# AdamCodd/local-hyperDB

Measured on AMD Instinct MI355X. Metric: queries/sec, N=10M d=384 fp16 top-100 (single-query stream; p50 latency alongside), higher is better.
Workload: dtype f16; 1 GPU; N=10000000 d=384 fp16 Q=1 cosine_similarity top-100, row-sharded x1; rows_per_gpu=10000000, accumulate=f32, exchange=none

## Files before the change

### local-hyperdb_amd/csrc/hdb_api.hip

```cpp
#include "hdb_common.h"
#include "hdb_quant.h"
#include "hdb_ws.h"
#include "hdb_plan.h"
#include "hdb_group_plan.h"
#include "hdb_devbuf.h"
#include "../../include/hyperdb_hip.h"
#include <string>
#include <cmath>
#include <cstring>
#include <cstdio>
#include <algorithm>
#include <vector>
#include <chrono>
#include <atomic>

static thread_local std::string g_err;
static int fail(int code, const std::string& msg) { g_err = msg; return code; }
#define HIP_TRY(expr)                                                                              \
    do {                                                                                           \
        hipError_t e_ = (expr);                                                                    \
        if (e_ != hipSuccess)                                                                      \
            return fail(HDB_ERR_HIP, std::string(#expr) + ": " + hipGetErrorString(e_));           \
    } while (0)
#define LAUNCH_TRY(expr)                                                                           \
// ... 101 lines not shown
struct CacheBufs { DevBuf<float> inv, sq; };
static int caches_alloc(int64_t rows, CacheBufs& c) {
    HIP_TRY(c.inv.alloc((size_t)rows));
    HIP_TRY(c.sq.alloc((size_t)rows));
    return HDB_OK;
}
static void caches_commit(hdb_index* ix, CacheBufs& c) {
    if (!c.inv) return;
    ix->inv_norm.swap(c.inv); ix->sqnorm.swap(c.sq);
}

static double quant_gamma(int d) {
    const double u = std::ldexp(1.0, -24), m = (double)(d + 8) * u;
    return m / (1.0 - m) * (1.0 + std::ldexp(1.0, -20));
}
static double quant_gamma_m(int d) { return (double)(d + 8) * std::ldexp(1.0, -22); }
static double quant_gamma_rows(int d) { return std::max(quant_gamma(d), quant_gamma_m(d)); }
static size_t row_pitch(const hdb_index* ix) { return (size_t)hdb_row_bytes(ix->dtype, ix->d); }
#define HDB_QSTAT_WORDS 4
static hipError_t qstat_alloc(hdb_index* ix, hipStream_t st) {
    if (ix->qstat) return hipSuccess;
    const hipError_t e = ix->qstat.alloc(HDB_QSTAT_WORDS);
    return e != hipSuccess ? e : hipMemsetAsync(ix->qstat, 0, HDB_QSTAT_WORDS * sizeof(int), st);
}
static void plane_free(hdb_index* ix) { ix->pnib.reset(); ix->pbit.reset(); ix->prec.reset(); }
static void quant_free(hdb_index* ix) {
    ix->qcodes.reset(); ix->qaux.reset(); ix->q_rows = 0;
    plane_free(ix);
}
static size_t plane_row_bytes(int P) { return (size_t)hdb_quant_plane_units(P) * 20 + 16; }
static bool plane_alloc(hdb_index* ix, int64_t rows) {
    const size_t U = (size_t)hdb_quant_plane_units(ix->qP);
    DevBuf<uint8_t> nib; DevBuf<uint32_t> bit; DevBuf<float> rec;
    if (nib.alloc((size_t)rows * U * 16) != hipSuccess || bit.alloc((size_t)rows * U) != hipSuccess || rec.alloc((size_t)rows * 4) != hipSuccess) {
        (void)hipGetLastError();
        return false;
    }
    ix->pnib.swap(nib); ix->pbit.swap(bit); ix->prec.swap(rec);
    return true;
}
static int plane_rows(hdb_index* ix, int64_t row0, int64_t m, hipStream_t st) {
    if (!plane_possible(ix->d) || ix->plane_declined) return HDB_OK;
    if (!ix->pnib && !plane_wanted(ix->d, ix->opt)) return HDB_OK;
    if (!ix->pnib) {
        size_t free_b = 0, total_b = 0;
        if (hipMemGetInfo(&free_b, &total_b) != hipSuccess) { (void)hipGetLastError(); ix->plane_declined = true; return HDB_OK; }
        if (free_b < (size_t)ix->q_rows * plane_row_bytes(ix->qP) + ((size_t)1 << 30)) { ix->plane_declined = true; return HDB_OK; }
        if (!plane_alloc(ix, ix->q_rows)) { ix->plane_declined = true; return HDB_OK; }
        ix->pU = hdb_quant_plane_units(ix->qP);
        m = row0 + m; row0 = 0;
    }
    LAUNCH_TRY(hdb_launch_quant_plane_rows(ix->qcodes, ix->qaux, row0, m, ix->d, ix->qP, ix->pnib, ix->pbit, ix->prec, st));
    return HDB_OK;
}
struct ShadowBufs { DevBuf<int8_t> codes; DevBuf<float> aux; int64_t rows = 0; };
static int quant_alloc(const hdb_index* ix, int64_t rows, ShadowBufs& s) {
    hipError_t e = s.codes.alloc((size_t)rows * ix->qP);
    if (e == hipSuccess) e = s.aux.alloc((size_t)rows * 3);
    if (e != hipSuccess) return fail(HDB_ERR_NOMEM, std::string("the int8 shadow: ") + hipGetErrorString(e));
    s.rows = rows;
    return HDB_OK;
}
static int quant_room(const hdb_index* ix, int64_t need, bool tight, ShadowBufs& s) {
    if (need <= ix->q_rows && ix->qcodes) return HDB_OK;
    return quant_alloc(ix, tight ? need + 64 : need + need / 2 + 64, s);
}
static void quant_commit(hdb_index* ix, ShadowBufs& s) {
    if (!s.rows) return;
    ix->qcodes.swap(s.codes); ix->qaux.swap(s.aux); ix->q_rows = s.rows;
    plane_free(ix);
}
static int quant_reserve(hdb_index* ix, int64_t need, int64_t keep, hipStream_t st, bool tight = false) {
    ShadowBufs s;
    const int rc = quant_room(ix, need, tight, s);
    if (rc || !s.rows) return rc;
    if (keep > 0 && ix->qcodes) {
        HIP_TRY(hipMemcpyAsync(s.codes, ix->qcodes, (size_t)keep * ix->qP, hipMemcpyDeviceToDevice, st));
        HIP_TRY(hipMemcpyAsync(s.aux, ix->qaux, (size_t)keep * 3 * sizeof(float), hipMemcpyDeviceToDevice, st));
    }
    quant_commit(ix, s);
    return HDB_OK;
}
static int quant_rows(hdb_index* ix, int64_t row0, int64_t m, hipStream_t st) {
    if (m <= 0) return HDB_OK;
    const char* src = (const char*)ix->V + (size_t)row0 * row_pitch(ix);
// ... 1511 lines not shown
```

### local-hyperdb_amd/csrc/hdb_caps.h

```cpp
#pragma once
#include "../../include/hyperdb_hip.h"

static inline int hdb_scan_auto_blocks(int dtype, int row_bytes, bool vec, bool wide_rows) {
    if ((dtype == HDB_F8E4M3 || dtype == HDB_I8) && vec && (row_bytes == 256 || row_bytes == 384 || row_bytes == 512)) {
        const int b = 512 * 768 / row_bytes;
        return b < 1024 ? b : 1024;
    }
    return wide_rows ? 256 : 512;
}

#define HDB_BSCAN_TABLE_BYTES (60 * 1024)
static inline int hdb_bscan_qt(int d) {
    if (d <= 0 || d % 32 != 0) return -1;
    for (int qt = 4; qt >= 1; qt >>= 1)
        if ((int64_t)qt * 16 * d <= HDB_BSCAN_TABLE_BYTES) return qt;
    return (int64_t)8 * d <= HDB_BSCAN_TABLE_BYTES ? 0 : -1;
}
static inline int hdb_bscan_lds_bytes(int d, int qt) { return qt > 0 ? qt * 16 * d : 8 * d; }
static inline int hdb_bscan_auto_blocks(int d, int qt, int cus) {
    int per_cu = (160 * 1024) / (hdb_bscan_lds_bytes(d, qt) + 5 * 1024);
    per_cu = per_cu < 1 ? 1 : per_cu > 8 ? 8 : per_cu;
    return per_cu * (cus > 0 ? cus : 1);
}

// ... 206 lines not shown
    if (max_blocks > 0 && max_blocks < limit) limit = max_blocks;
    return hdb_grid_for((nwalk + 1) / 2, 4, (int)limit);
}
static inline int hdb_quant_plane_dbg_blocks(int64_t ntiles, int max_blocks) { return hdb_grid_for((ntiles + 1) / 2, 4, max_blocks > 0 ? max_blocks : 1024); }
struct HdbSkipPos { uint32_t w, o; };
struct HdbSkipStep { uint32_t dw, dn, step; };
__host__ __device__ __forceinline__ uint32_t hdb_plane_skip_count(uint32_t ntiles, uint32_t s_tiles) { return ntiles - s_tiles; }
__host__ __device__ __forceinline__ HdbSkipStep hdb_plane_skip_step(uint32_t step, uint32_t stride) {
    const uint32_t m = stride - 1u;
    HdbSkipStep s;
    s.dw = m ? step / m : 0u; s.dn = m ? step % m : 0u; s.step = step;
    return s;
}
__host__ __device__ __forceinline__ HdbSkipPos hdb_plane_skip_start(uint32_t tp, uint32_t s_tiles, uint32_t stride) {
    const uint32_t m = stride - 1u;
    HdbSkipPos p;
    const uint32_t w = m ? tp / m : s_tiles;
    if (w < s_tiles) { p.w = w; p.o = tp - w * m; }
    else { p.w = s_tiles; p.o = tp - s_tiles * m; }
    return p;
}
__host__ __device__ __forceinline__ void hdb_plane_skip_advance(HdbSkipPos& p, const HdbSkipStep& s, uint32_t s_tiles, uint32_t stride) {
    if (p.w >= s_tiles) { p.o += s.step; return; }
    const uint32_t m = stride - 1u;
    p.w += s.dw; p.o += s.dn;
    if (p.o >= m) { p.o -= m; ++p.w; }
    if (p.w >= s_tiles) { p.o += (p.w - s_tiles) * m; p.w = s_tiles; }
}
__host__ __device__ __forceinline__ int64_t hdb_plane_skip_tile(const HdbSkipPos& p, uint32_t s_tiles, uint32_t stride) {
    if (p.w >= s_tiles) return (int64_t)s_tiles * stride + p.o;
    const uint32_t jit = (uint32_t)(hdb_tile_index((int64_t)p.w, (int64_t)stride) - (int64_t)p.w * stride);
    return (int64_t)p.w * stride + p.o + (p.o >= jit ? 1u : 0u);
}

static inline int hdb_qb_supported(int d) { return d == 128 || d == 256 || d == 384 || d == 512; }
static inline void qb_shape(int nq, int& wq, int& nqt) {
    const int tq = (nq + 15) / 16;
    wq = tq <= 4 ? 1 : tq <= 8 ? 2 : 4;
    nqt = (tq + wq - 1) / wq;
}
static inline int hdb_qb_scan_blocks(int64_t ntiles, int nq, int cus, int max_blocks) {
    int wq, nqt; qb_shape(nq, wq, nqt);
    const int64_t lim = max_blocks > 0 ? max_blocks : 2 * (int64_t)cus;
    return hdb_grid_for(ntiles, 4 / wq, (int)(lim < 512 ? lim : 512));
}
static inline int64_t hdb_qb_slots(int blocks, int nq) { int wq, nqt; qb_shape(nq, wq, nqt); return (int64_t)blocks * (4 / wq) * 4; }
```

### local-hyperdb_amd/csrc/hdb_launch.h

```cpp
#pragma once
#include <stddef.h>
#include <stdint.h>

struct ScanArgs;
struct FusedArgs;
struct BatchArgs;
struct BitsArgs;
struct QuantArgs;

#define HDB_ANYD_DECL(name) int name(const ScanArgs* args, int dpad, int mode, int nq_launch, const void* q, const float* sqnorm, \
                                     const float* qsq, const float* qscl, int blocks, void* stream)
#define HDB_GEOM_DECL(name) int name(const ScanArgs* args, int mode, int nq_launch, const void* q16, const float* sqnorm, \
                                     const float* qsq, const float* qscl, int blocks, int variant, void* stream, const BatchArgs* f)

extern "C" {
int hdb_launch_scan(const ScanArgs* args, int dtype, int mode, int nq_launch, int max_blocks, void* stream);
int hdb_launch_list_rows(unsigned long long* cand, const uint32_t* cnt, uint32_t cap, int nq, const int64_t* rows, int64_t m, void* stream);
int hdb_launch_rownorm(const void* V, int64_t n, int d, int dtype, float* inv_norm, float* sqnorm, int* nan_flag, void* stream);
int hdb_launch_qprep(const void* Q, int nq, int d, bool f64, float* qinv, float* qsq, int* qnan, void* q16, float* qscl, void* stream);
int hdb_launch_qprep2(const void* Q, int nq, int d, bool f64, float* qinv, float* qsq, int* qnan, void* q16, float* qscl,
                      float* thr_init, uint32_t* cnt_init, uint32_t* qbits, int W, void* stream);
int hdb_launch_signpack(const void* V, int64_t n, int d, int dtype, int64_t row0, uint32_t* bits, void* stream);
int hdb_launch_qsign(const void* Q, int nq, int d, bool f64, int W, uint32_t* qbits, void* stream);
int hdb_launch_hamming(const ScanArgs* args, int mode, int nq_launch, const uint32_t* bits, int64_t npad, int W,
// ... 74 lines not shown
int hdb_launch_mfma_kslice_bf16(const ScanArgs* a, int dslice, int mode, int nq_launch, const void* q, const float* sqnorm,
                                const float* qsq, int blocks, void* stream);
int hdb_launch_mfma_kslice_bf16_wide(const ScanArgs* a, int dslice, int mode, int nq_launch, const void* q, const float* sqnorm,
                                     const float* qsq, int blocks, void* stream);
int hdb_launch_mfma_kslice_f8(const ScanArgs* a, int dslice, int mode, int nq_launch, const void* q, const float* sqnorm,
                              const float* qsq, int blocks, void* stream);
int hdb_launch_mfma_kslice_f8_wide(const ScanArgs* a, int dslice, int mode, int nq_launch, const void* q, const float* sqnorm,
                                   const float* qsq, int blocks, void* stream);
int hdb_launch_mfma_scan_f8_lds(const ScanArgs* args, int mode, int nq_launch, const void* q, const float* sqnorm,
                                const float* qsq, int blocks, void* stream);
int hdb_launch_mfma_scan_f8_lds_wide(const ScanArgs* args, int mode, int nq_launch, const void* q, const float* sqnorm,
                                     const float* qsq, int blocks, void* stream);
int hdb_launch_mfma_kslice_f8_lds(const ScanArgs* a, int dslice, int mode, int nq_launch, const void* q, const float* sqnorm,
                                  const float* qsq, int blocks, void* stream);
int hdb_launch_mfma_kslice_f8_lds_wide(const ScanArgs* a, int dslice, int mode, int nq_launch, const void* q, const float* sqnorm,
                                       const float* qsq, int blocks, void* stream);
HDB_ANYD_DECL(hdb_launch_mfma_anyd_a); HDB_ANYD_DECL(hdb_launch_mfma_anyd_b);
HDB_ANYD_DECL(hdb_launch_mfma_anyd_c); HDB_ANYD_DECL(hdb_launch_mfma_anyd_d);
HDB_ANYD_DECL(hdb_launch_mfma_anyd_e); HDB_ANYD_DECL(hdb_launch_mfma_anyd_f);

size_t hdb_mfma_fused_ctl_bytes(void);
int hdb_launch_mfma_fused(const ScanArgs* args, int dtype, const FusedArgs* fa, int max_blocks, void* stream);
int hdb_launch_mfma_fused_wide(const ScanArgs* args, const FusedArgs* fa, int blocks, void* stream);
int hdb_launch_bits_fused(const BitsArgs* args, int jaccard, int max_blocks, void* stream);
int hdb_launch_l1_tile(const ScanArgs* args, int dtype, int mode, int nq_launch, int max_blocks, void* stream);

int hdb_launch_quant_rows(const void* V, int64_t n, int d, int dtype, int P, int8_t* codes, float* aux, int* nan_flag, double gamma,
                          void* stream);
int hdb_launch_quant_gather(const int8_t* codes, const float* aux, const int64_t* rows, int64_t m, int P, int8_t* codes_out,
                            float* aux_out, void* stream);
int hdb_launch_quant_qprep(const float* Q, int nq, int d, int P, int8_t* qcodes, float* qaux, int* stat, uint32_t* pl_cnt, void* stream);
int hdb_launch_quant_qprep_m(const float* Q, int nq, int d, int P, float* qinv, float* qsq, int* qnan, void* q16, float* qscl,
                             int8_t* qcodes, float* qaux, int* stat, uint32_t* cnt_init, uint32_t* pl_cnt, void* stream);
int hdb_launch_quant_plane_rows(const int8_t* codes, const float* aux, int64_t row0, int64_t m, int d, int P, uint8_t* nib, uint32_t* bitw,
                                float* rec, void* stream);
int hdb_launch_quant_plane_scan(const QuantArgs* args, int dbg, int blocks, void* stream);
int hdb_launch_quant_scan(const QuantArgs* args, int mode, int max_blocks, void* stream);
int hdb_launch_quant_scan_one(const QuantArgs* args, int mode, int max_blocks, void* stream);
int hdb_launch_quant_rescore(const void* V, int d, int dtype, const float* Q, int nq, int metric, const float* inv_norm,
                             const float* qinv, const float* bias, const uint8_t* mask, unsigned long long* cand,
                             const uint32_t* cnt, uint32_t cap, void* stream);
int hdb_launch_quant_finalize(const unsigned long long* cand, const uint32_t* cnt, uint32_t cap, int nq, uint32_t k, uint32_t kk,
                              int64_t row_base, int64_t* idx_out, float* score_out, int32_t* status, const int* qnan,
                              const float* qaux, const float* thr, int* stat, unsigned long long* cand_rw, const float* sc, int64_t ld,
                              void* stream);

int hdb_launch_rerank_prep(const int64_t* cand, int m, int nq, int64_t n, int64_t row_base, const uint8_t* mask, const int* qnan,
                           int64_t* rows, uint32_t* cnt, int32_t* status, void* stream);
int hdb_launch_rerank_score(const ScanArgs* args, int dtype, int nq_launch, void* stream);

int hdb_launch_group_collapse(const int64_t* idx, const float* score, int nq, int m, int k, const int32_t* groups, int64_t n_groups,
                              int64_t n, int64_t row_base, int64_t* idx_out, float* score_out, const int32_t* status_in,
                              int32_t* status_out, int carry, void* stream);
int hdb_launch_group_best(const float* scores, int64_t n, int64_t ld, int nq, const int32_t* groups, int64_t n_groups,
                          unsigned long long* best, void* stream);
int hdb_launch_group_demote(float* scores, int64_t n, int64_t ld, int nq, const int32_t* groups, int64_t n_groups,
                            const unsigned long long* best, int* bad, void* stream);
int hdb_launch_group_finish(int64_t* idx, const float* score, int nq, int k, int32_t* status, const int* bad, void* stream);

int hdb_launch_qb_scan(const QuantArgs* args, int mode, float* wstat, int64_t wld, int max_blocks, void* stream);
int hdb_launch_qb_thr(const float* vals, int64_t n, int64_t ld, int nq, uint32_t m, float* thr, void* stream);
int hdb_launch_qb_rescore(const void* V, int d, const void* q16, const float* qscl, const float* qinv, const float* inv_norm,
                          const float* bias, const uint8_t* mask, int metric, unsigned long long* cand, const uint32_t* cnt,
                          uint32_t cap, int nq, void* stream);
}
```

### local-hyperdb_amd/csrc/hdb_quant.hip

```cpp
#include "hdb_common.h"
#include "hdb_quant.h"
#include "hdb_finalize.h"
#include "../../include/hyperdb_hip.h"

__device__ __forceinline__ float hq_up(double x) {
    x = x * (1.0 + 0x1p-40);
    float f = (float)x;
    if ((double)f < x) f = nextafterf(f, INFINITY);
    return f;
}

__device__ __forceinline__ float hq_f(__half v) { return __half2float(v); }
__device__ __forceinline__ float hq_f(hdb_bf16 v) { return hdb_bf16_to_f(v); }
__device__ __forceinline__ float hq_f(float v) { return v; }

template <typename T> struct HqElem;
template <> struct HqElem<__half> { static constexpr int EPC = 8; };
template <> struct HqElem<hdb_bf16> { static constexpr int EPC = 8; };
template <> struct HqElem<float> { static constexpr int EPC = 4; };

__device__ __forceinline__ void hq_unpack(const uint4& raw, float (&x)[8], __half*) {
    const __half2* h = reinterpret_cast<const __half2*>(&raw);
#pragma unroll
    for (int i = 0; i < 4; ++i) { float2 f = __half22float2(h[i]); x[2 * i] = f.x; x[2 * i + 1] = f.y; }
// ... 461 lines not shown
        const int64_t r0 = hdb_tile_index(t, a.tile_stride) * 16 + 4 * g;
        const int64_t rr[4] = {r0, r0 + 1, r0 + 2, r0 + 3};
        const int u_own = hdb_owned_row(l16);
        const int64_t row = r0 + u_own;
        const int64_t out_i = t * 16 + 4 * g + u_own;
        const bool live = hq_rows4_bounds<NQ, NJ, (NJ > 0 ? NJ : 2)>(a, qs, qc, rr, l16, row, [&](int q, float lo, float hi, bool masked) {
            if (MODE == 2) {
                a.dbg[row] = hi;
            } else if (MODE == 0) {
                if (a.nsub > 0) wbest[q] = max(wbest[q], hdb_f2key(lo));
                else a.scores[(int64_t)q * a.ld + out_i] = lo;
                if (NQ == 1 && a.pl_hi) a.pl_hi[out_i] = hi;
            } else if (!masked && !qc.bad[q] && hi >= q_thr[q]) {
                hq_emit(stage, q, hi, row);
            }
        });
        if (MODE == 0 && a.nsub == 0 && !live && (l16 & 3) == 0)
#pragma unroll
            for (int q = 0; q < NQ; ++q) a.scores[(int64_t)q * a.ld + out_i] = -INFINITY;
        if (MODE == 0 && NQ == 1 && a.pl_hi && !live && (l16 & 3) == 0) a.pl_hi[out_i] = -INFINITY;
    }
    if (MODE == 0 && a.nsub > 0) {
#pragma unroll
        for (int q = 0; q < NQ; ++q) {
            uint32_t wm = wbest[q];
#pragma unroll
            for (int o = 32; o > 0; o >>= 1) wm = max(wm, (uint32_t)__shfl_xor((int)wm, o, 64));
            if (lane == 0) a.wmax[(int64_t)q * a.nsub + blockIdx.x * 4 + wave] = wm;
        }
    }
    if (MODE == 1) hq_stage_flush<NQ>(stage);
}

__global__ __launch_bounds__(256) void hdb_quant_plane_rows_kernel(const int8_t* codes, const float* aux, int64_t row0, int64_t m, int d, int P,
                                                                   int U, uint8_t* nib, uint32_t* bitw, float* rec) {
    const int lane = threadIdx.x & 63, g = lane >> 4, l16 = lane & 15;
    const int64_t wave = ((int64_t)blockIdx.x * 256 + threadIdx.x) >> 6;
    const int64_t nwaves = ((int64_t)gridDim.x * 256) >> 6;
    for (int64_t base = wave * 4; base < m; base += nwaves * 4) {
        const int64_t r = row0 + base + g;
        const bool valid = base + g < m;
        int ss = 0;
        if (valid && l16 < U) {
            const int8_t* src = codes + r * (int64_t)P + 32 * l16;
            uint4 raw[2];
            raw[0] = *reinterpret_cast<const uint4*>(src);
            raw[1] = (32 * l16 + 16 < P) ? *reinterpret_cast<const uint4*>(src + 16) : make_uint4(0u, 0u, 0u, 0u);
            const uint32_t* cw = reinterpret_cast<const uint32_t*>(raw);
            uint32_t nw[4] = {0u, 0u, 0u, 0u}, bw = 0u;
#pragma unroll
            for (int w = 0; w < 8; ++w) {
#pragma unroll
                for (int b = 0; b < 4; ++b) {
                    const int c = (int)(int8_t)((cw[w] >> (8 * b)) & 0xFFu);
                    const int h = c >> 3;
                    const uint32_t u5 = (uint32_t)(h + 16);
                    const int rho = c - (8 * h + 4);
                    if (32 * l16 + 4 * w + b < d) ss += rho * rho;
                    nw[w >> 1] |= (u5 >> 1) << (8 * b + 4 * (w & 1));
                    bw |= (u5 & 1u) << (8 * b + w);
                }
            }
            *reinterpret_cast<uint4*>(nib + (r * (int64_t)U + l16) * 16) = make_uint4(nw[0], nw[1], nw[2], nw[3]);
            bitw[r * (int64_t)U + l16] = bw;
        }
#pragma unroll
        for (int o = 8; o > 0; o >>= 1) ss += __shfl_xor(ss, o, 64);
        if (valid && l16 == 0) {
            const float R = sqrtf((float)ss) * (1.f + 0x1p-20f);
            *reinterpret_cast<float4*>(rec + 4 * r) = make_float4(aux[3 * r + HDB_QROW_S], aux[3 * r + HDB_QROW_E], aux[3 * r + HDB_QROW_T], R);
        }
    }
}

#define HQ_PL_QUEUE 48
template <int J, bool DBG>
__global__ __launch_bounds__(256) __attribute__((amdgpu_num_sgpr(96))) void hdb_quant_plane_scan_kernel(QuantArgs a) {
    extern __shared__ __attribute__((aligned(16))) char smem[];
    int4* qs = reinterpret_cast<int4*>(smem);
    __shared__ int part[4][2][64 * J];
    __shared__ HqStage stage;
    __shared__ uint32_t queue[4][HQ_PL_QUEUE];
    __shared__ uint32_t surv_cnt;
    const int U = a.pl_units, nch = a.P >> 4;
    if (threadIdx.x < 4) stage.cnt[threadIdx.x] = 0u;
    if (threadIdx.x == 0) surv_cnt = 0u;
    for (int i = threadIdx.x; i < 2 * U; i += 256) qs[i] = i < nch ? reinterpret_cast<const int4*>(a.qcodes)[i] : make_int4(0, 0, 0, 0);
    const float* qo = a.qaux;
    const float q_s = qo[HDB_QQ_S], q_n = qo[HDB_QQ_N], q_d = qo[HDB_QQ_D], q_cn = qo[HDB_QQ_CN];
    const int q_cs = (int)qo[HDB_QQ_CS];
    const bool q_bad = qo[HDB_QQ_BAD] != 0.f;
    const bool cosine = a.metric == HDB_COSINE;
    const float q_inv = cosine ? a.qinv[0] : 1.f;
    float thr1[1] = {(!DBG && a.nsub == 0) ? a.thr[0] : 0.f};
    __syncthreads();
    if (!DBG && a.nsub > 0) hq_fold_thr<1>(a, thr1);
    const float q_thr = thr1[0];

    const int lane = threadIdx.x & 63, wave = __builtin_amdgcn_readfirstlane(threadIdx.x >> 6);
    const int npieces = 16 * U;
    int qoff[J];
#pragma unroll
    for (int j = 0; j < J; ++j) {
        const int f = lane + 64 * j;
        qoff[j] = f < npieces ? 2 * (f % U) : 0;
    }
    const float absmin = 0x1p-100f * (float)(a.d + 8);
    typedef unsigned int u32x4 __attribute__((ext_vector_type(4)));
    typedef float f32x4 __attribute__((ext_vector_type(4)));
    const int64_t ntiles = a.ntiles;
    const int et = lane >> 4, er = lane & 15;
    int qn = 0;
    uint32_t nsurv = 0u;
    auto drain = [&](int base, int m) {
        const QuantArgs& a = hq_args_in_memory();
        HqQuery<1> qc;
        qc.s[0] = q_s; qc.n[0] = q_n; qc.d[0] = q_d; qc.sq[0] = 0.f; qc.inv[0] = q_inv; qc.bad[0] = q_bad;
        int ln = lane;
        asm volatile("" : "+v"(ln));
        const int g = ln >> 4, l16 = ln & 15;
        int64_t rr[4];
#pragma unroll
        for (int u = 0; u < 4; ++u) rr[u] = 4 * g + u < m ? (int64_t)queue[wave][base + 4 * g + u] : a.n;
        const int own = 4 * g + hdb_owned_row(l16);
        const int64_t row = own < m ? (int64_t)queue[wave][base + own] : a.n;
        hq_rows4_bounds<1, 0, 1>(a, qs, qc, rr, l16, row, [&](int, float, float hi, bool masked) {
            if (!masked && !q_bad && hi >= q_thr) hq_emit(stage, 0, hi, row);
        });
    };

    const uint32_t s_tiles = DBG ? 0u : a.pl_s_tiles, s_stride = DBG ? 1u : a.pl_s_stride;
    const uint32_t nwalk = hdb_plane_skip_count((uint32_t)ntiles, s_tiles);
    const uint32_t tp0 = ((uint32_t)blockIdx.x * 4u + (uint32_t)wave) * 2u;
    const HdbSkipStep sk_step = hdb_plane_skip_step((uint32_t)gridDim.x * 8u, s_stride), sk_next = {0u, 1u, 1u};
    HdbSkipPos pos = hdb_plane_skip_start(tp0 < nwalk ? tp0 : 0u, s_tiles, s_stride);
    for (uint32_t tp = tp0; tp < nwalk; tp += (uint32_t)gridDim.x * 8u, hdb_plane_skip_advance(pos, sk_step, s_tiles, s_stride)) {
        int64_t tl[2];
        {
            HdbSkipPos p1 = pos;
            hdb_plane_skip_advance(p1, sk_next, s_tiles, s_stride);
            tl[0] = hdb_plane_skip_tile(pos, s_tiles, s_stride);
            tl[1] = tp + 1u < nwalk ? hdb_plane_skip_tile(p1, s_tiles, s_stride) : ntiles;
        }
        u32x4 nv[2][J];
        uint32_t bv[2][J];
        int ln = lane;
        asm volatile("" : "+v"(ln));
#pragma unroll
        for (int tt = 0; tt < 2; ++tt) {
            const int pieces_left = (int)min((int64_t)16, max((int64_t)0, a.n - tl[tt] * 16)) * U;
            const uint8_t* nb = a.pl_nib + tl[tt] * (int64_t)npieces * 16;
            const uint32_t* bb = a.pl_bit + tl[tt] * (int64_t)npieces;
#pragma unroll
            for (int j = 0; j < J; ++j) {
                if (ln < pieces_left - 64 * j) {
                    nv[tt][j] = __builtin_nontemporal_load(reinterpret_cast<const u32x4*>(nb + (uint32_t)ln * 16u) + 64 * j);
                    bv[tt][j] = __builtin_nontemporal_load(bb + (uint32_t)ln + 64 * j);
                } else {
                    nv[tt][j] = u32x4{0u, 0u, 0u, 0u};
                    bv[tt][j] = 0u;
                }
            }
        }
        const int64_t row = (et ? tl[1] : tl[0]) * 16 + er;
        const bool rvalid = lane < 32 && row < a.n;
        f32x4 rc = f32x4{0.f, 0.f, 0.f, 0.f};
        float invn = 1.f, bias = 0.f;
        bool masked = false;
        if (rvalid) {
            rc = __builtin_nontemporal_load(reinterpret_cast<const f32x4*>(a.pl_rec) + row);
            if (cosine) invn = a.inv_norm[row];
            if (a.bias) bias = a.bias[row];
            if (a.mask) masked = !a.mask[row];
        }
        __builtin_amdgcn_sched_barrier(0);
#pragma unroll
        for (int j = 0; j < J; ++j) {
            const int4 x = qs[qoff[j]], y = qs[qoff[j] + 1];
            const int qw[8] = {x.x, x.y, x.z, x.w, y.x, y.y, y.z, y.w};
#pragma unroll
            for (int tt = 0; tt < 2; ++tt) {
                const uint32_t bw = bv[tt][j];
                const uint32_t w4[4] = {nv[tt][j].x, nv[tt][j].y, nv[tt][j].z, nv[tt][j].w};
                int s = 0;
#pragma unroll
                for (int i = 0; i < 4; ++i) {
                    const uint32_t lo = ((w4[i] << 1) & 0x1E1E1E1Eu) | ((bw >> (2 * i)) & 0x01010101u);
                    const uint32_t hi = ((w4[i] >> 3) & 0x1E1E1E1Eu) | ((bw >> (2 * i + 1)) & 0x01010101u);
                    s = __builtin_amdgcn_sdot4((int)lo, qw[2 * i], s, false);
                    s = __builtin_amdgcn_sdot4((int)hi, qw[2 * i + 1], s, false);
                }
                part[wave][tt][lane + 64 * j] = s;
            }
            __builtin_amdgcn_sched_barrier(0);
        }
        __builtin_amdgcn_fence(__ATOMIC_RELEASE, "wavefront");
        __builtin_amdgcn_wave_barrier();
        __builtin_amdgcn_fence(__ATOMIC_ACQUIRE, "wavefront");
        int S = 0;
        if (lane < 32)
            for (int i = 0; i < U; ++i) S += part[wave][et][er * U + i];
        __builtin_amdgcn_fence(__ATOMIC_RELEASE, "wavefront");
        __builtin_amdgcn_wave_barrier();
        float hi5 = -INFINITY;
        const bool dead = !rvalid || masked || q_bad;
        if (!dead) {
            const float fc = (float)(8 * S - 124 * q_cs);
            const float Uf = q_cn * rc.w;
            float ch = fc + Uf, cl = fc - Uf;
            ch = ch + (fabsf(ch) * 0x1p-20f + 1.f);
            cl = cl - (fabsf(cl) * 0x1p-20f + 1.f);
            const float k = q_s * rc.x;
            const float A5 = k * ch, Al = k * cl;
            const float Amax = fmaxf(fabsf(A5), fabsf(Al));
            const float c0 = (q_n * rc.y + q_d * rc.z) * (1.f + 0x1p-10f);
            const float B5 = c0 + fabsf(A5) * 0x1p-10f + absmin;
            const float Bmax = c0 + Amax * 0x1p-10f + absmin;
            const float Mx = Amax + Bmax;
            float X = (A5 + B5) + (Mx * 0x1p-18f + 1e-30f);
            float mM = Mx * (1.f + 0x1p-17f);
            if (cosine) { X = X * invn * q_inv; mM = mM * invn * q_inv; }
            const float Z = mM + fabsf(bias);
            float h = X;
            if (a.bias) h += bias;
            hi5 = h + (Z * 0x1p-18f + 4e-30f);
            if (hi5 != hi5) hi5 = INFINITY;
        }
        if (DBG) {
            if (rvalid) a.dbg[row] = hi5;
            continue;
        }
        const bool keep = !dead && !(hi5 < q_thr);
        const unsigned long long km = __ballot(keep);
        if (km == 0ull) continue;
        if (keep) queue[wave][qn + __popcll(km & ((1ull << lane) - 1ull))] = (uint32_t)row;
        const int nk = __popcll(km);
        qn += nk; nsurv += (uint32_t)nk;
        __builtin_amdgcn_fence(__ATOMIC_RELEASE, "wavefront");
        __builtin_amdgcn_wave_barrier();
        __builtin_amdgcn_fence(__ATOMIC_ACQUIRE, "wavefront");
        if (qn >= 16) {
            do { qn -= 16; drain(qn, 16); } while (qn >= 16);
            __builtin_amdgcn_fence(__ATOMIC_RELEASE, "wavefront");
            __builtin_amdgcn_wave_barrier();
        }
    }
    if (!DBG) {
        if (s_tiles != 0u) {
            const QuantArgs& am = hq_args_in_memory();
            const uint32_t nslots = s_tiles * 16u, dslot = (uint32_t)gridDim.x * 256u;
            uint32_t cbase = ((uint32_t)blockIdx.x * 4u + (uint32_t)wave) * 64u;
            float hnext = cbase + lane < nslots ? am.pl_hi[cbase + lane] : 0.f;
#pragma unroll 1
            for (; cbase < nslots; cbase += dslot) {
// ... 166 lines not shown
    const int nch = a.P >> 4;
    const int nj = (nch + 15) >> 4;
    if (nj == 1) hipLaunchKernelGGL((hdb_quant_scan_kernel<MODE, NQ, 1>), dim3(blocks), dim3(256), lds, st, a);
    else if (nj == 2) hipLaunchKernelGGL((hdb_quant_scan_kernel<MODE, NQ, 2>), dim3(blocks), dim3(256), lds, st, a);
    else if (nj == 3) hipLaunchKernelGGL((hdb_quant_scan_kernel<MODE, NQ, 3>), dim3(blocks), dim3(256), lds, st, a);
    else hipLaunchKernelGGL((hdb_quant_scan_kernel<MODE, NQ, 0>), dim3(blocks), dim3(256), lds, st, a);
}
template <int MODE>
static void hq_launch_scan_mode(const QuantArgs& a, int blocks, size_t lds, hipStream_t st) {
    switch (a.nq) {
    case 1: hq_launch_scan_nq<MODE, 1>(a, blocks, lds, st); break;
    case 2: hq_launch_scan_nq<MODE, 2>(a, blocks, lds, st); break;
    case 3: hq_launch_scan_nq<MODE, 3>(a, blocks, lds, st); break;
    default: hq_launch_scan_nq<MODE, 4>(a, blocks, lds, st); break;
    }
}
static bool hq_copy_args_ok(const QuantArgs& a) {
    return !a.G || (a.V && a.row_bytes > 0 && a.row_bytes % 16 == 0 && (reinterpret_cast<uintptr_t>(a.V) & 15) == 0 && (reinterpret_cast<uintptr_t>(a.G) & 15) == 0);
}
extern "C" int hdb_launch_quant_scan(const QuantArgs* args, int mode, int max_blocks, void* stream) {
    const QuantArgs& a = *args;
    if (a.nq < 1 || a.nq > 4 || (a.P & 15) != 0) return (int)hipErrorInvalidValue;
    const size_t lds = (size_t)a.nq * a.P;
    const int blocks = hdb_quant_scan_blocks(a.ntiles, max_blocks);
    if (a.nsub != 0 && (a.nsub > HDB_QUANT_NSUB_MAX || !a.wmax || (mode == 0 ? a.nsub != 4 * blocks : !a.thr_out))) return (int)hipErrorInvalidValue;
    if (mode == 0) hq_launch_scan_mode<0>(a, blocks, lds, (hipStream_t)stream);
    else {
        if (!hq_copy_args_ok(a)) return (int)hipErrorInvalidValue;
        hq_launch_scan_mode<1>(a, blocks, lds, (hipStream_t)stream);
    }
    return (int)hipGetLastError();
}

extern "C" int hdb_launch_quant_plane_rows(const int8_t* codes, const float* aux, int64_t row0, int64_t m, int d, int P, uint8_t* nib,
                                           uint32_t* bitw, float* rec, void* stream) {
    if (m <= 0) return 0;
    const int U = hdb_quant_plane_units(P);
    if (U > 16 || (P & 15) != 0) return (int)hipErrorInvalidValue;
    hipLaunchKernelGGL(hdb_quant_plane_rows_kernel, dim3(hdb_grid_for(m, 16, 8192)), dim3(256), 0, (hipStream_t)stream, codes, aux, row0, m, d,
                       P, U, nib, bitw, rec);
    return (int)hipGetLastError();
}
extern "C" int hdb_launch_quant_plane_scan(const QuantArgs* args, int dbg, int blocks, void* stream) {
    const QuantArgs& a = *args;
    const int U = a.pl_units;
    if (blocks < 1 || blocks > (1 << 22)) return (int)hipErrorInvalidValue;
    if (a.nq != 1 || U < 1 || U > 16 || U != hdb_quant_plane_units(a.P) || (a.metric != HDB_DOT && a.metric != HDB_COSINE)) return (int)hipErrorInvalidValue;
    if (!dbg && a.nsub != 0 && (a.nsub > HDB_QUANT_NSUB_MAX || !a.wmax || !a.thr_out)) return (int)hipErrorInvalidValue;
    if (!dbg && (!a.cnt || !a.cand || !a.pl_cnt || !hq_copy_args_ok(a))) return (int)hipErrorInvalidValue;
    if (a.ntiles < 0 || a.ntiles > 0x10000000) return (int)hipErrorInvalidValue;
    if (!dbg && a.pl_s_tiles != 0u && (!a.pl_hi || a.pl_s_stride < 1u || (uint64_t)a.pl_s_tiles * a.pl_s_stride > (uint64_t)a.ntiles)) return (int)hipErrorInvalidValue;
    const size_t lds = (size_t)U * 32;
    hipStream_t st = (hipStream_t)stream;
    const int J = hdb_quant_plane_j(U);
#define HQ_PLANE(J_) do { if (dbg) hipLaunchKernelGGL((hdb_quant_plane_scan_kernel<J_, true>), dim3(blocks), dim3(256), lds, st, a); \
                          else hipLaunchKernelGGL((hdb_quant_plane_scan_kernel<J_, false>), dim3(blocks), dim3(256), lds, st, a); } while (0)
    if (J == 1) HQ_PLANE(1); else if (J == 2) HQ_PLANE(2); else if (J == 3) HQ_PLANE(3); else HQ_PLANE(4);
#undef HQ_PLANE
    return (int)hipGetLastError();
}
extern "C" int hdb_launch_quant_scan_one(const QuantArgs* args, int mode, int max_blocks, void* stream) {
    const QuantArgs& a = *args;
    if (a.nq != 1 || (a.P & 15) != 0 || a.nsub != 0 || mode != 2 || !a.dbg) return (int)hipErrorInvalidValue;
    const size_t lds = (size_t)a.P;
    const int blocks = hdb_quant_scan_blocks(a.ntiles, max_blocks);
    const int nj = ((a.P >> 4) + 15) >> 4;
    hipStream_t st = (hipStream_t)stream;
#define HQ_ONE(NJ_) hipLaunchKernelGGL((hdb_quant_scan_kernel<2, 1, NJ_>), dim3(blocks), dim3(256), lds, st, a)
    if (nj == 1) HQ_ONE(1); else if (nj == 2) HQ_ONE(2); else if (nj == 3) HQ_ONE(3); else HQ_ONE(0);
#undef HQ_ONE
    return (int)hipGetLastError();
}

// ... 43 lines not shown
```

Measured before the change: 2064 queries/s.

## Pack per-row plane records into compressed per-tile blocks with precomputed cosine scaling

Replaces the 16-byte float4 per-row record (scale, err terms, residual radius) with a 256-byte per-16-row tile block. Each block holds bf16-rounded-up scale codes, 8-bit residual radius codes and tile-max error terms, in separate dot and cosine flavours where inv_norm is already folded in. This is meant to cut the scan's per-row loads from 16 bytes plus an inv_norm read to about 3 bytes plus one shared tile vector. In exchange the bound gets looser: tile-max error terms and rounded-up k and radius widen the candidate bound. The rows kernel also now works per tile and needs extra encoding work.

```diff
diff --git a/local-hyperdb_amd/csrc/hdb_api.hip b/local-hyperdb_amd/csrc/hdb_api.hip
--- a/local-hyperdb_amd/csrc/hdb_api.hip
+++ b/local-hyperdb_amd/csrc/hdb_api.hip
@@ -157,7 +157,8 @@
 static bool plane_alloc(hdb_index* ix, int64_t rows) {
     const size_t U = (size_t)hdb_quant_plane_units(ix->qP);
     DevBuf<uint8_t> nib; DevBuf<uint32_t> bit; DevBuf<float> rec;
-    if (nib.alloc((size_t)rows * U * 16) != hipSuccess || bit.alloc((size_t)rows * U) != hipSuccess || rec.alloc((size_t)rows * 4) != hipSuccess) {
+    if (nib.alloc((size_t)rows * U * 16) != hipSuccess || bit.alloc((size_t)rows * U) != hipSuccess ||
+        rec.alloc((size_t)hdb_plane_rec_bytes(rows) / sizeof(float)) != hipSuccess) {
         (void)hipGetLastError();
         return false;
     }
@@ -175,7 +176,10 @@
         ix->pU = hdb_quant_plane_units(ix->qP);
         m = row0 + m; row0 = 0;
     }
-    LAUNCH_TRY(hdb_launch_quant_plane_rows(ix->qcodes, ix->qaux, row0, m, ix->d, ix->qP, ix->pnib, ix->pbit, ix->prec, st));
+    if (m <= 0) return HDB_OK;
+    const int64_t rows = std::max(ix->n, row0 + m);
+    LAUNCH_TRY(hdb_launch_quant_plane_rows(ix->qcodes, ix->qaux, ix->inv_norm, row0 / 16, (row0 + m + 15) / 16, rows, ix->d, ix->qP, ix->pnib,
+                                           ix->pbit, ix->prec, st));
     return HDB_OK;
 }
 struct ShadowBufs { DevBuf<int8_t> codes; DevBuf<float> aux; int64_t rows = 0; };
diff --git a/local-hyperdb_amd/csrc/hdb_caps.h b/local-hyperdb_amd/csrc/hdb_caps.h
--- a/local-hyperdb_amd/csrc/hdb_caps.h
+++ b/local-hyperdb_amd/csrc/hdb_caps.h
@@ -262,6 +262,46 @@
     const uint32_t jit = (uint32_t)(hdb_tile_index((int64_t)p.w, (int64_t)stride) - (int64_t)p.w * stride);
     return (int64_t)p.w * stride + p.o + (p.o >= jit ? 1u : 0u);
 }
+#define HDB_PLANE_TILE_BYTES 256
+#define HDB_PLANE_BLOCK_BYTES 64
+#define HDB_PLANE_BLOCK_DOT 0
+#define HDB_PLANE_BLOCK_COSINE 1
+#define HDB_PLANE_BLOCK_K 0
+#define HDB_PLANE_BLOCK_RC 32
+#define HDB_PLANE_BLOCK_TILE 48
+__host__ __device__ __forceinline__ int64_t hdb_plane_rec_bytes(int64_t rows) { return (rows + 15) / 16 * HDB_PLANE_TILE_BYTES; }
+__host__ __device__ __forceinline__ int64_t hdb_plane_block_off(int64_t tile, int flavour) {
+    return tile * HDB_PLANE_TILE_BYTES + (int64_t)flavour * HDB_PLANE_BLOCK_BYTES;
+}
+__host__ __device__ __forceinline__ float hdb_plane_bits_f(uint32_t u) { union { uint32_t u; float f; } c; c.u = u; return c.f; }
+__host__ __device__ __forceinline__ uint32_t hdb_plane_f_bits(float f) { union { uint32_t u; float f; } c; c.f = f; return c.u; }
+__host__ __device__ __forceinline__ uint16_t hdb_plane_k_encode(double k) {
+    if (!(k > 0.0)) return k == k ? (uint16_t)0 : (uint16_t)0x7FC0;
+    float f = (float)k;
+    if (f != f || f - f != 0.f) return (uint16_t)0x7F80;
+    uint32_t h = hdb_plane_f_bits(f) >> 16;
+    if ((double)hdb_plane_bits_f(h << 16) < k) ++h;
+    return (uint16_t)h;
+}
+__host__ __device__ __forceinline__ float hdb_plane_k_hi(uint32_t code) { return hdb_plane_bits_f(code << 16); }
+__host__ __device__ __forceinline__ float hdb_plane_k_lo(float k_hi) {
+    return k_hi >= 0x1p-126f && k_hi <= 0x1.fep127f ? k_hi * (1.f - 0x1p-7f) : 0.f;
+}
+__host__ __device__ __forceinline__ uint32_t hdb_plane_rc_encode(uint32_t ss) {
+    const uint32_t t = 4u * ss;
+    uint32_t rc = (uint32_t)sqrtf((float)t);
+    while (rc * rc < t) ++rc;
+    while (rc > 0u && (rc - 1u) * (rc - 1u) >= t) --rc;
+    return rc < 255u ? rc : 255u;
+}
+__host__ __device__ __forceinline__ float hdb_plane_rc_decode(uint32_t rc) { return 0.5f * (float)rc; }
+__host__ __device__ __forceinline__ float hdb_plane_up(double x) {
+    if (!(x > 0.0)) return x == x ? 0.f : hdb_plane_bits_f(0x7F800000u);
+    float f = (float)x;
+    if (f != f || f - f != 0.f) return hdb_plane_bits_f(0x7F800000u);
+    if ((double)f < x) f = hdb_plane_bits_f(hdb_plane_f_bits(f) + 1u);
+    return f;
+}
 
 static inline int hdb_qb_supported(int d) { return d == 128 || d == 256 || d == 384 || d == 512; }
 static inline void qb_shape(int nq, int& wq, int& nqt) {
diff --git a/local-hyperdb_amd/csrc/hdb_launch.h b/local-hyperdb_amd/csrc/hdb_launch.h
--- a/local-hyperdb_amd/csrc/hdb_launch.h
+++ b/local-hyperdb_amd/csrc/hdb_launch.h
@@ -130,8 +130,8 @@
 int hdb_launch_quant_qprep(const float* Q, int nq, int d, int P, int8_t* qcodes, float* qaux, int* stat, uint32_t* pl_cnt, void* stream);
 int hdb_launch_quant_qprep_m(const float* Q, int nq, int d, int P, float* qinv, float* qsq, int* qnan, void* q16, float* qscl,
                              int8_t* qcodes, float* qaux, int* stat, uint32_t* cnt_init, uint32_t* pl_cnt, void* stream);
-int hdb_launch_quant_plane_rows(const int8_t* codes, const float* aux, int64_t row0, int64_t m, int d, int P, uint8_t* nib, uint32_t* bitw,
-                                float* rec, void* stream);
+int hdb_launch_quant_plane_rows(const int8_t* codes, const float* aux, const float* inv_norm, int64_t t0, int64_t t1, int64_t n, int d, int P,
+                                uint8_t* nib, uint32_t* bitw, float* rec, void* stream);
 int hdb_launch_quant_plane_scan(const QuantArgs* args, int dbg, int blocks, void* stream);
 int hdb_launch_quant_scan(const QuantArgs* args, int mode, int max_blocks, void* stream);
 int hdb_launch_quant_scan_one(const QuantArgs* args, int mode, int max_blocks, void* stream);
diff --git a/local-hyperdb_amd/csrc/hdb_quant.hip b/local-hyperdb_amd/csrc/hdb_quant.hip
--- a/local-hyperdb_amd/csrc/hdb_quant.hip
+++ b/local-hyperdb_amd/csrc/hdb_quant.hip
@@ -517,43 +517,82 @@
     if (MODE == 1) hq_stage_flush<NQ>(stage);
 }
 
-__global__ __launch_bounds__(256) void hdb_quant_plane_rows_kernel(const int8_t* codes, const float* aux, int64_t row0, int64_t m, int d, int P,
-                                                                   int U, uint8_t* nib, uint32_t* bitw, float* rec) {
+__global__ __launch_bounds__(256) void hdb_quant_plane_rows_kernel(const int8_t* codes, const float* aux, const float* inv_norm, int64_t t0,
+                                                                   int64_t t1, int64_t n, int d, int P, int U, uint8_t* nib,
+                                                                   uint32_t* bitw, float* rec) {
     const int lane = threadIdx.x & 63, g = lane >> 4, l16 = lane & 15;
     const int64_t wave = ((int64_t)blockIdx.x * 256 + threadIdx.x) >> 6;
     const int64_t nwaves = ((int64_t)gridDim.x * 256) >> 6;
-    for (int64_t base = wave * 4; base < m; base += nwaves * 4) {
-        const int64_t r = row0 + base + g;
-        const bool valid = base + g < m;
+    for (int64_t t = t0 + wave; t < t1; t += nwaves) {
+        int ssr[4];
+#pragma unroll
+        for (int it = 0; it < 4; ++it) {
+            const int64_t r = t * 16 + 4 * it + g;
+            int ss = 0;
+            if (r < n && l16 < U) {
+                const int8_t* src = codes + r * (int64_t)P + 32 * l16;
+                uint4 raw[2];
+                raw[0] = *reinterpret_cast<const uint4*>(src);
+                raw[1] = (32 * l16 + 16 < P) ? *reinterpret_cast<const uint4*>(src + 16) : make_uint4(0u, 0u, 0u, 0u);
+                const uint32_t* cw = reinterpret_cast<const uint32_t*>(raw);
+                uint32_t nw[4] = {0u, 0u, 0u, 0u}, bw = 0u;
+#pragma unroll
+                for (int w = 0; w < 8; ++w) {
+#pragma unroll
+                    for (int b = 0; b < 4; ++b) {
+                        const int c = (int)(int8_t)((cw[w] >> (8 * b)) & 0xFFu);
+                        const int h = c >> 3;
+                        const uint32_t u5 = (uint32_t)(h + 16);
+                        const int rho = c - (8 * h + 4);
+                        if (32 * l16 + 4 * w + b < d) ss += rho * rho;
+                        nw[w >> 1] |= (u5 >> 1) << (8 * b + 4 * (w & 1));
+                        bw |= (u5 & 1u) << (8 * b + w);
+                    }
+                }
+                *reinterpret_cast<uint4*>(nib + (r * (int64_t)U + l16) * 16) = make_uint4(nw[0], nw[1], nw[2], nw[3]);
+                bitw[r * (int64_t)U + l16] = bw;
+            }
+#pragma unroll
+            for (int o = 8; o > 0; o >>= 1) ss += __shfl_xor(ss, o, 64);
+            ssr[it] = ss;
+        }
         int ss = 0;
-        if (valid && l16 < U) {
-            const int8_t* src = codes + r * (int64_t)P + 32 * l16;
-            uint4 raw[2];
-            raw[0] = *reinterpret_cast<const uint4*>(src);
-            raw[1] = (32 * l16 + 16 < P) ? *reinterpret_cast<const uint4*>(src + 16) : make_uint4(0u, 0u, 0u, 0u);
-            const uint32_t* cw = reinterpret_cast<const uint32_t*>(raw);
-            uint32_t nw[4] = {0u, 0u, 0u, 0u}, bw = 0u;
-#pragma unroll
-            for (int w = 0; w < 8; ++w) {
-#pragma unroll
-                for (int b = 0; b < 4; ++b) {
-                    const int c = (int)(int8_t)((cw[w] >> (8 * b)) & 0xFFu);
-                    const int h = c >> 3;
-                    const uint32_t u5 = (uint32_t)(h + 16);
-                    const int rho = c - (8 * h + 4);
-                    if (32 * l16 + 4 * w + b < d) ss += rho * rho;
-                    nw[w >> 1] |= (u5 >> 1) << (8 * b + 4 * (w & 1));
-                    bw |= (u5 & 1u) << (8 * b + w);
-                }
-            }
-            *reinterpret_cast<uint4*>(nib + (r * (int64_t)U + l16) * 16) = make_uint4(nw[0], nw[1], nw[2], nw[3]);
-            bitw[r * (int64_t)U + l16] = bw;
-        }
-#pragma unroll
-        for (int o = 8; o > 0; o >>= 1) ss += __shfl_xor(ss, o, 64);
-        if (valid && l16 == 0) {
-            const float R = sqrtf((float)ss) * (1.f + 0x1p-20f);
-            *reinterpret_cast<float4*>(rec + 4 * r) = make_float4(aux[3 * r + HDB_QROW_S], aux[3 * r + HDB_QROW_E], aux[3 * r + HDB_QROW_T], R);
+#pragma unroll
+        for (int it = 0; it < 4; ++it) {
+            const int v = __shfl(ssr[it], 16 * (lane & 3), 64);
+            if (((lane >> 2) & 3) == it) ss = v;
+        }
+        const int64_t r = t * 16 + l16;
+        const bool valid = lane < 16 && r < n;
+        const double absmin = 0x1p-100 * (double)(d + 8);
+        double kd = 0.0, kc = 0.0;
+        float ed = 0.f, td = 0.f, fd = 0.f, ec = 0.f, tc = 0.f, fc = 0.f;
+        uint32_t rcode = 0u;
+        if (valid) {
+            const float s = aux[3 * r + HDB_QROW_S], e = aux[3 * r + HDB_QROW_E], tt = aux[3 * r + HDB_QROW_T];
+            const double inv = (double)inv_norm[r];
+            kd = (double)s; kc = (double)s * inv;
+            ed = e; td = tt; fd = hdb_plane_up(absmin);
+            ec = hdb_plane_up((double)e * inv); tc = hdb_plane_up((double)tt * inv); fc = hdb_plane_up(absmin * inv * (1.0 + 0x1p-40));
+            rcode = hdb_plane_rc_encode((uint32_t)ss);
+        }
+#pragma unroll
+        for (int o = 8; o > 0; o >>= 1) {
+            ed = fmaxf(ed, __shfl_xor(ed, o, 64)); td = fmaxf(td, __shfl_xor(td, o, 64)); fd = fmaxf(fd, __shfl_xor(fd, o, 64));
+            ec = fmaxf(ec, __shfl_xor(ec, o, 64)); tc = fmaxf(tc, __shfl_xor(tc, o, 64)); fc = fmaxf(fc, __shfl_xor(fc, o, 64));
+        }
+        if (lane < 16) {
+            char* tile = reinterpret_cast<char*>(rec) + hdb_plane_block_off(t, 0);
+#pragma unroll
+            for (int fl = 0; fl < 2; ++fl) {
+                char* blk = tile + fl * HDB_PLANE_BLOCK_BYTES;
+                reinterpret_cast<uint16_t*>(blk + HDB_PLANE_BLOCK_K)[l16] = hdb_plane_k_encode(fl == HDB_PLANE_BLOCK_COSINE ? kc : kd);
+                reinterpret_cast<uint8_t*>(blk + HDB_PLANE_BLOCK_RC)[l16] = (uint8_t)rcode;
+                if (l16 == 0)
+                    *reinterpret_cast<float4*>(blk + HDB_PLANE_BLOCK_TILE) =
+                        fl == HDB_PLANE_BLOCK_COSINE ? make_float4(ec, tc, fc, 0.f) : make_float4(ed, td, fd, 0.f);
+            }
+            if (l16 < 8) *reinterpret_cast<uint4*>(tile + 2 * HDB_PLANE_BLOCK_BYTES + 16 * l16) = make_uint4(0u, 0u, 0u, 0u);
         }
     }
 }
@@ -590,9 +629,8 @@
         const int f = lane + 64 * j;
         qoff[j] = f < npieces ? 2 * (f % U) : 0;
     }
-    const float absmin = 0x1p-100f * (float)(a.d + 8);
     typedef unsigned int u32x4 __attribute__((ext_vector_type(4)));
-    typedef float f32x4 __attribute__((ext_vector_type(4)));
+    typedef float f32x3 __attribute__((ext_vector_type(3)));
     const int64_t ntiles = a.ntiles;
     const int et = lane >> 4, er = lane & 15;
     int qn = 0;
@@ -649,12 +687,15 @@
         }
         const int64_t row = (et ? tl[1] : tl[0]) * 16 + er;
         const bool rvalid = lane < 32 && row < a.n;
-        f32x4 rc = f32x4{0.f, 0.f, 0.f, 0.f};
-        float invn = 1.f, bias = 0.f;
+        f32x3 tm = f32x3{0.f, 0.f, 0.f};
+        uint32_t kcode = 0u, rcode = 0u;
+        float bias = 0.f;
         bool masked = false;
         if (rvalid) {
-            rc = __builtin_nontemporal_load(reinterpret_cast<const f32x4*>(a.pl_rec) + row);
-            if (cosine) invn = a.inv_norm[row];
+            const char* blk = reinterpret_cast<const char*>(a.pl_rec) + hdb_plane_block_off(et ? tl[1] : tl[0], cosine ? HDB_PLANE_BLOCK_COSINE : HDB_PLANE_BLOCK_DOT);
+            kcode = reinterpret_cast<const uint16_t*>(blk + HDB_PLANE_BLOCK_K)[er];
+            rcode = reinterpret_cast<const uint8_t*>(blk + HDB_PLANE_BLOCK_RC)[er];
+            tm = *reinterpret_cast<const f32x3*>(blk + HDB_PLANE_BLOCK_TILE);
             if (a.bias) bias = a.bias[row];
             if (a.mask) masked = !a.mask[row];
         }
@@ -691,20 +732,23 @@
         const bool dead = !rvalid || masked || q_bad;
         if (!dead) {
             const float fc = (float)(8 * S - 124 * q_cs);
-            const float Uf = q_cn * rc.w;
+            const float Uf = q_cn * hdb_plane_rc_decode(rcode);
             float ch = fc + Uf, cl = fc - Uf;
             ch = ch + (fabsf(ch) * 0x1p-20f + 1.f);
             cl = cl - (fabsf(cl) * 0x1p-20f + 1.f);
-            const float k = q_s * rc.x;
-            const float A5 = k * ch, Al = k * cl;
+            const float k_hi = hdb_plane_k_hi(kcode), k_lo = hdb_plane_k_lo(k_hi);
+            float k_up = q_s * k_hi, k_dn = q_s * k_lo;
+            k_up = k_up + k_up * 0x1p-20f;
+            k_dn = k_dn - k_dn * 0x1p-20f;
+            const float A5 = (ch >= 0.f ? k_up : k_dn) * ch, Al = (cl >= 0.f ? k_dn : k_up) * cl;
             const float Amax = fmaxf(fabsf(A5), fabsf(Al));
-            const float c0 = (q_n * rc.y + q_d * rc.z) * (1.f + 0x1p-10f);
-            const float B5 = c0 + fabsf(A5) * 0x1p-10f + absmin;
-            const float Bmax = c0 + Amax * 0x1p-10f + absmin;
+            const float c0 = (q_n * tm.x + q_d * tm.y) * (1.f + 0x1p-10f);
+            const float B5 = c0 + fabsf(A5) * 0x1p-10f + tm.z;
+            const float Bmax = c0 + Amax * 0x1p-10f + tm.z;
             const float Mx = Amax + Bmax;
             float X = (A5 + B5) + (Mx * 0x1p-18f + 1e-30f);
             float mM = Mx * (1.f + 0x1p-17f);
-            if (cosine) { X = X * invn * q_inv; mM = mM * invn * q_inv; }
+            if (cosine) { X = X * q_inv; mM = mM * q_inv; }
             const float Z = mM + fabsf(bias);
             float h = X;
             if (a.bias) h += bias;
@@ -937,13 +981,13 @@
     return (int)hipGetLastError();
 }
 
-extern "C" int hdb_launch_quant_plane_rows(const int8_t* codes, const float* aux, int64_t row0, int64_t m, int d, int P, uint8_t* nib,
-                                           uint32_t* bitw, float* rec, void* stream) {
-    if (m <= 0) return 0;
+extern "C" int hdb_launch_quant_plane_rows(const int8_t* codes, const float* aux, const float* inv_norm, int64_t t0, int64_t t1, int64_t n, int d,
+                                           int P, uint8_t* nib, uint32_t* bitw, float* rec, void* stream) {
+    if (t1 <= t0) return 0;
     const int U = hdb_quant_plane_units(P);
-    if (U > 16 || (P & 15) != 0) return (int)hipErrorInvalidValue;
-    hipLaunchKernelGGL(hdb_quant_plane_rows_kernel, dim3(hdb_grid_for(m, 16, 8192)), dim3(256), 0, (hipStream_t)stream, codes, aux, row0, m, d,
-                       P, U, nib, bitw, rec);
+    if (U > 16 || (P & 15) != 0 || t0 < 0 || (t1 - 1) * 16 >= n) return (int)hipErrorInvalidValue;
+    hipLaunchKernelGGL(hdb_quant_plane_rows_kernel, dim3(hdb_grid_for(t1 - t0, 4, 8192)), dim3(256), 0, (hipStream_t)stream, codes, aux, inv_norm,
+                       t0, t1, n, d, P, U, nib, bitw, rec);
     return (int)hipGetLastError();
 }
 extern "C" int hdb_launch_quant_plane_scan(const QuantArgs* args, int dbg, int blocks, void* stream) {
```

Result: faster. 2124 queries/s (median of 6 runs) (+2.9%).
